# rgl-epfl/large-steps-pytorch

Measured on AMD Instinct MI355X. Metric: from_differential_solves_per_sec, higher is better.
Workload: dtype f32; 1 GPU; cfg4_plane1m: 1000x1000 plane, V=1000000, nnz(M)=6992002, M=I+50*L_uniform, u=M v, k=3, factor once (not timed), re-solve timed; method=nested-dissection, device=AMD Radeon Graphics

## Files before the change

large-steps-pytorch_amd/csrc/direct.hip:

```cpp
#include "common.h"
#include <vector>
#include <chrono>
#include <algorithm>
#include <atomic>
#include <string.h>
#include <memory>
#include <mutex>

namespace ls {

struct alignas(64) Tile {
    int store;
    int row0, s, b, own_start, bnd_off, front_off;
    int leaf;
    int pfront_off, cix;
    int forward;
    int arity;
    long long finv_off, w_off;
};

static_assert(sizeof(Tile) == 64, "Tile layout");
__device__ __forceinline__ Tile load_tile(const Tile* __restrict__ tiles, int idx) {
    const int lane = threadIdx.x & 63;
    const int w = lane < 16 ? reinterpret_cast<const int*>(tiles)[(size_t)idx * 16 + lane] : 0;
// ... 1128 lines not shown
        p.s_cap = std::max(p.s_cap, T.nd[i].s); p.b_cap = std::max(p.b_cap, T.nd[i].b);
        red_up = std::max(red_up, T.nd[i].s); red_down = std::max(red_down, T.nd[i].s + T.nd[i].b);
    }
    p.up_b = red_up >= long_up; p.down_b = red_down >= env.long_red;
    const int up_bw = std::min(ND_BW, red_up >= 1400 ? 8 : 4), down_bw = std::min(ND_BW, red_down >= 1400 ? 8 : 4);
    p.up_nw = p.up_b ? up_bw : pick_nw(red_up, 32); p.down_nw = p.down_b ? down_bw : pick_nw(red_down, env.steps);
    int64_t rows_up = 0, rows_down = 0;
    for (int64_t i = a0; i < a1; ++i) { rows_up += T.nd[i].b; rows_down += T.nd[i].s; }
    auto pick_chunks = [&](int64_t rows, int bw) {
        int c = 4;
        while (c > 1 && rows / (ND_ROWS * bw * c) < 500) --c;
        return c;
    };
    p.up_chunks = pick_chunks(rows_up, up_bw);
    p.down_chunks = pick_chunks(rows_down, down_bw);
    const int up_rows = p.up_b ? ND_ROWS * up_bw * p.up_chunks : WAVE, down_rows = p.down_b ? ND_ROWS * down_bw * p.down_chunks : WAVE;
    const size_t up_s_bytes = ((size_t)p.s_cap * p.b_cap + (size_t)p.s_cap * kmax) * sizeof(float);
    p.up_s = p.b_cap <= 256 && p.s_cap <= 256 && up_s_bytes <= 40 * 1024 && !env.no_small;
    if (p.up_s) { p.up_b = 0; p.up_nw = std::max(1, div_up(p.b_cap, WAVE)); }
    p.up_p = !env.no_pack && p.b_cap <= WAVE && p.s_cap <= 256 && lv > 0;
    p.down_p = !env.no_pack && p.s_cap <= WAVE / 2;
    auto pack_level = [&](bool up_sweep, int& first, int& count, int& lds_rows_s, int& lds_rows_b) {
        first = (int)T.ptiles.size();
        lds_rows_s = lds_rows_b = 0;
        int64_t i = a0;
        while (i < a1) {
            PackedTile t;
            memset(&t, 0, sizeof(t));
            t.leaf = lv + 1 >= T.levels; t.arity = T.arity;
            int rows = 0;
            while (i < a1 && t.n < ND_PACK) {
                const NodeD& nd = T.nd[i];
                const int r = up_sweep ? nd.b : nd.s;
                if (t.n && rows + r > WAVE) break;
                NodeP& q = t.d[t.n];
                q.s = nd.s; q.b = nd.b; q.own_start = nd.own_start; q.bnd_off = nd.bnd_off; q.front_off = nd.front_off;
                q.pfront_off = nd.pfront_off; q.cix = nd.cix; q.pad = 0; q.finv_off = nd.finv_off; q.w_off = nd.w_off;
                t.row0[t.n + 1] = t.row0[t.n] + r;
                t.sb0[t.n + 1] = t.sb0[t.n] + nd.s;
                t.sx0[t.n + 1] = t.sx0[t.n] + nd.b;
                rows += r; ++t.n; ++i;
            }
            for (int c = t.n + 1; c <= ND_PACK; ++c) { t.row0[c] = t.row0[t.n]; t.sb0[c] = t.sb0[t.n]; t.sx0[c] = t.sx0[t.n]; }
            lds_rows_s = std::max(lds_rows_s, t.sb0[t.n]); lds_rows_b = std::max(lds_rows_b, t.sx0[t.n]);
            T.ptiles.push_back(t);
        }
        count = (int)T.ptiles.size() - first;
    };
    int dummy = 0;
    if (p.up_p) { pack_level(true, p.up_p_first, p.up_p_tiles, p.up_p_lds, dummy); p.up_s = 0; p.up_b = 0; }
    if (p.down_p) { pack_level(false, p.down_p_first, p.down_p_tiles, p.down_p_s, p.down_p_lds); p.down_b = 0; }
    p.up_first = (int)tiles.size();
    const int up_threads = WAVE * p.up_nw;
    std::vector<int> up_nodes;
    for (int64_t i = a0; i < a1; ++i) {
        const bool store_tiles = !p.up_s && T.nd[i].s > 2 * up_threads;
        const int rows = std::max(T.nd[i].b, (T.nd[i].s && !store_tiles) ? 1 : 0);
        for (int r = 0; r < rows; r += (p.up_s ? 1 << 30 : up_rows)) {
            tiles.push_back(tile_of(i, r, 0));
            tiles.back().store = (r == 0 && !store_tiles) ? 1 : 0;
            up_nodes.push_back((int)(i - a0));
        }
        if (store_tiles)
            for (int r = 0; r < T.nd[i].s; r += up_threads) { tiles.push_back(tile_of(i, r, 0)); tiles.back().store = 2; up_nodes.push_back((int)(i - a0)); }
    }
    auto xcd_order = [&](int first, std::vector<int>& node_of_tile) {
        const int n = (int)tiles.size() - first;
        if (a1 - a0 < 8 || n < 16) return;
        std::vector<std::vector<Tile>> bucket(8);
        for (int t = 0; t < n; ++t) bucket[(size_t)(node_of_tile[(size_t)t] & 7)].push_back(tiles[(size_t)(first + t)]);
        size_t longest = 0;
        for (auto& bk : bucket) longest = std::max(longest, bk.size());
        Tile idle;
        memset(&idle, 0, sizeof(idle));
        idle.store = 3; idle.forward = 2;
        tiles.resize((size_t)first);
        for (size_t r = 0; r < longest; ++r)
            for (int x = 0; x < 8; ++x) tiles.push_back(r < bucket[(size_t)x].size() ? bucket[(size_t)x][r] : idle);
    };
    xcd_order(p.up_first, up_nodes);
    p.up_tiles = (int)tiles.size() - p.up_first;
    p.down_first = (int)tiles.size();
    std::vector<int> down_nodes;
    for (int64_t i = a0; i < a1; ++i)
        for (int r = 0; r < T.nd[i].s; r += down_rows) { tiles.push_back(tile_of(i, r, 0)); down_nodes.push_back((int)(i - a0)); }
    if (lv + 1 < T.levels)
        for (int64_t i = a0; i < a1; ++i)
            for (int r = 0; r < T.nd[i].b; r += WAVE * p.down_nw) { tiles.push_back(tile_of(i, r, 1)); down_nodes.push_back((int)(i - a0)); }
    xcd_order(p.down_first, down_nodes);
    p.down_tiles = (int)tiles.size() - p.down_first;
    return ((size_t)p.s_cap + p.b_cap + 16 * WAVE) * kmax * sizeof(float);
}

void account_index_bytes(const CreatePlan& T, ls_direct* d) {
    const int levels = T.levels, arity = T.arity;
    d->lvl_idx_up.assign((size_t)levels, 0); d->lvl_idx_down.assign((size_t)levels, 0);
    std::vector<int64_t> fpos((size_t)levels, 0), bsum((size_t)levels + 1, 0);
    for (int lv = 0; lv < levels; ++lv)
        for (int64_t i = T.level_off[lv]; i < T.level_off[lv + 1]; ++i)
            if (T.active(i, lv)) { fpos[(size_t)lv] += T.nd[i].s + T.nd[i].b; bsum[(size_t)lv] += T.nd[i].b; }
    for (int lv = 0; lv < d->tier_root; ++lv) {
        const LevelPlan& p = d->plan[lv];
        d->lvl_idx_up[(size_t)lv] = (p.up_p ? (int64_t)p.up_p_tiles * (int64_t)sizeof(PackedTile) : (int64_t)p.up_tiles * (int64_t)sizeof(Tile)) + fpos[(size_t)lv] + 4 * bsum[(size_t)lv];
        d->lvl_idx_down[(size_t)lv] = (p.down_p ? (int64_t)p.down_p_tiles * (int64_t)sizeof(PackedTile) : (int64_t)p.down_tiles * (int64_t)sizeof(Tile)) + 4 * fpos[(size_t)lv] +
                                      4 * bsum[(size_t)lv + 1];
    }
    if (d->tier_root >= levels) return;
    const int H = levels - d->tier_root;
    for (const TierWG& g : T.wgs)
        for (int ph = 0; ph < H; ++ph) {
            d->lvl_idx_up[(size_t)(levels - 1 - ph)] += (int64_t)(g.up_off[ph + 1] - g.up_off[ph]) * (int64_t)sizeof(TierItem);
            d->lvl_idx_down[(size_t)(d->tier_root + ph)] += (int64_t)(g.down_off[ph + 1] - g.down_off[ph]) * (int64_t)sizeof(TierItem);
        }
    d->lvl_idx_up[(size_t)d->tier_root] += (int64_t)T.wgs.size() * (int64_t)sizeof(TierWG);
    d->lvl_idx_down[(size_t)d->tier_root] += (int64_t)T.wgs.size() * (int64_t)sizeof(TierWG);
    for (int lv = d->tier_root; lv < levels; ++lv) {
        const bool inner = lv + 1 < levels;
        if (inner) d->lvl_idx_up[(size_t)lv] += 4 * (int64_t)arity * fpos[(size_t)lv];
        if (lv == d->tier_root || !inner) d->lvl_idx_up[(size_t)lv] += 4 * bsum[(size_t)lv];
        if (inner) d->lvl_idx_down[(size_t)lv] += 4 * fpos[(size_t)lv] + 4 * bsum[(size_t)lv + 1];
    }
    const int64_t q0 = T.sub_lo * T.span(T.cut, d->tier_root);
    double mx[2] = {0, 0}, sum[2] = {0, 0};
    for (size_t w = 0; w < T.wgs.size(); ++w) {
        double wu = 0, wd = 0;
        int64_t span = 1;
        for (int lv = d->tier_root; lv < levels; ++lv) {
            const int64_t first = T.level_off[lv] + (q0 + (int64_t)w) * span;
            for (int64_t i = first; i < first + span; ++i) {
                const NodeD& n = T.nd[i];
                const double s4 = (n.s + 3) & ~3, b4 = (n.b + 3) & ~3, tri_w = ((int64_t)n.s * (n.s + 1) / 2 + 3) & ~(int64_t)3;
                if (n.flags & NODE_SPARSE) { wu += tri_w + 3.0 * n.b; wd += tri_w + 3.0 * n.b; }
                else { wu += s4 * n.b; wd += (s4 + b4) * n.s; }
            }
            span *= arity;
        }
        mx[0] = std::max(mx[0], wu); mx[1] = std::max(mx[1], wd); sum[0] += wu; sum[1] += wd;
    }
    const double nw = (double)std::max<size_t>(T.wgs.size(), 1);
    d->tier_balance[0] = mx[0]; d->tier_balance[1] = sum[0] / nw; d->tier_balance[2] = mx[1]; d->tier_balance[3] = sum[1] / nw;
}

}

extern "C" int ls_direct_create(const ls_direct_arrays* A, int device, void* stream, ls_direct** out) {
    LS_REQUIRE(A && out, LS_E_INVALID, "ls_direct_create: null argument");
    LS_REQUIRE(A->tier_waves == 0 || A->tier_waves == TIER_WAVES || A->tier_waves == TIER_WAVES_WIDE || A->tier_waves == TIER_WAVES_FULL, LS_E_INVALID,
               "ls_direct_create: tier_waves must be 0 (library's rule), 4, 8 or 16");
    const int64_t V = A->V, n_bnd = A->n_bnd, n_front = A->n_front;
    const int levels = A->levels, arity = A->arity;
    LS_REQUIRE(A->h_nodes && A->h_perm && A->h_push_ptr && V > 0 && levels >= 1 && levels <= 30 && n_bnd >= 0 && n_front >= V &&
               (arity == 2 || arity == 4 || arity == 8), LS_E_INVALID, "ls_direct_create: bad argument");
    LS_REQUIRE(V < INT32_MAX && n_bnd < INT32_MAX && n_front * arity < INT32_MAX, LS_E_OVERFLOW, "ls_direct_create: plan exceeds int32 offsets");
    *out = nullptr;
    CreatePlan T{levels, arity};
    T.level_off.resize((size_t)levels + 1);
    {
        int64_t cnt = 1, off = 1;
        for (int lv = 0; lv <= levels; ++lv) {
            T.level_off[lv] = off; off += cnt; cnt *= arity;
            LS_REQUIRE(off < ((int64_t)1 << 30), LS_E_OVERFLOW, "ls_direct_create: tree too large");
        }
    }
    DeviceGuard g(device);
    LS_HIP(g.err);
    hipStream_t st = (hipStream_t)stream;
    const bool timing = env_plan_timing();
    const NdEnv env = nd_env();
    const auto t_create = std::chrono::steady_clock::now();
    auto lap = [&](const char* what) { if (timing) fprintf(stderr, "[ls_direct_create] %-28s %.2f ms\n", what, std::chrono::duration<double, std::milli>(std::chrono::steady_clock::now() - t_create).count()); };
    std::unique_ptr<ls_direct, int (*)(ls_direct*)> d(new ls_direct(), ls_direct_destroy);
    d->device = device; d->levels = levels; d->arity = arity; d->n_nodes = (int)(T.level_off[levels] - 1); d->V = V; d->n_bnd = n_bnd; d->n_front = n_front;
    d->finv = A->d_finv; d->wf = A->d_wf; d->wb = A->d_wb;
    d->u4 = A->d_u4; d->d4 = A->d_d4;
    d->tri = A->d_tri; d->sp_ptr = A->d_sp_ptr; d->sp_ent = (const SpEnt*)A->d_sp_ent;
    const int n_ranks = std::max(1, (int)A->shard_count), rank = std::min(std::max(0, (int)A->shard_rank), n_ranks - 1);
    int cut = 0;
    while (cut + 1 < levels && T.level_off[cut + 1] - T.level_off[cut] < n_ranks) ++cut;
    if (n_ranks == 1) cut = 0;
    const int64_t n_sub = T.level_off[cut + 1] - T.level_off[cut];
    T.sub_lo = n_sub * rank / n_ranks; T.sub_hi = n_sub * (rank + 1) / n_ranks;
    d->shard_rank = rank; d->shard_count = n_ranks; d->cut = T.cut = cut;
    T.mask.assign((size_t)n_front, 0);
    int rc = LS_OK;
    if ((rc = read_nodes(A, T, d.get())) || (rc = choose_tier(T, A->h_ppos, A->tier_waves, env, d.get()))) return rc;
    d->upper_lo = (d->tier_root < levels && d->tier_root > 0) ? T.nd[T.level_off[d->tier_root - 1]].own_start : (int)V;
    d->plan.resize(levels);
    size_t lds_max = 0;
    const int long_up = env.long_up > 0 ? env.long_up : levels >= 8 ? 256 : 64;
    for (int lv = 0; lv < d->tier_root; ++lv) lds_max = std::max(lds_max, plan_level(T, lv, long_up, env, d->kmax, d->plan[lv]));
    account_index_bytes(T, d.get());
    if (lds_max > LEVEL_LDS) {
        set_error("ls_direct_create: a front needs %zu bytes of LDS (separator too large for this kernel)", lds_max);
        return LS_E_INVALID;
    }
    if (n_ranks > 1 && cut >= 1) {
        d->exch_f0 = T.nd[T.level_off[cut - 1]].front_off;
        d->exch_f1 = T.nd[T.level_off[cut]].front_off;
    }
    if (n_ranks > 1) {
        d->owned_rows.assign((size_t)V, 0);
        for (int lv = 0; lv < levels; ++lv)
            for (int64_t i = T.level_off[lv]; i < T.level_off[lv + 1]; ++i)
                if (lv < cut ? rank == 0 : T.active(i, lv))
                    for (int r = 0; r < T.nd[i].s; ++r) d->owned_rows[(size_t)A->h_perm[T.nd[i].own_start + r]] = 1;
    }
    lap("tables built (host)");
    hipStream_t su = side_stream(device, 0);
    LS_REQUIRE(su, LS_E_STATE, "ls_direct_create: no side stream on this device");
    auto table = [&](void** dst, size_t bytes) -> hipError_t {
        size_t cap = bytes;
        *dst = pool_take(device, bytes, &cap);
        if (!*dst) { const hipError_t e = pool_alloc(device, dst, bytes); if (e != hipSuccess) return e; }
        d->tables.emplace_back(*dst, cap);
        return hipSuccess;
    };
    auto up = [&](auto** dst, const auto* src, size_t n) -> int {
        LS_HIP(table((void**)dst, std::max<size_t>(n, 1) * sizeof(**dst)));
        if (n) LS_HIP(hipMemcpyAsync(*dst, src, n * sizeof(**dst), hipMemcpyHostToDevice, su));
        return LS_OK;
    };
    if ((rc = up(&d->tiles, T.tiles.data(), T.tiles.size())) || (rc = up(&d->ptiles, T.ptiles.data(), T.ptiles.size())) ||
        (rc = up(&d->perm, A->h_perm, (size_t)V)) ||
        (rc = up(&d->ppos, A->h_ppos, (size_t)n_bnd)) || (rc = up(&d->push_ptr, A->h_push_ptr, (size_t)n_front + 1)) ||
        (rc = up(&d->push_tgt, A->h_push_tgt, (size_t)n_bnd)) || (rc = up(&d->mask, T.mask.data(), T.mask.size())) ||
        (rc = up(&d->d_items, T.items.data(), T.items.size())) || (rc = up(&d->pull, T.pull.data(), T.pull.size())) ||
        (rc = up(&d->d_wgs, T.wgs.data(), T.wgs.size())))
        return rc;
    hipError_t e = table((void**)&d->bp, sizeof(float) * (size_t)V * d->kmax);
    if (e == hipSuccess) e = table((void**)&d->braw, sizeof(float) * (size_t)V * d->kmax);
    if (e == hipSuccess) e = table((void**)&d->slots, sizeof(float) * (size_t)n_front * d->arity * d->kmax);
    if (e == hipSuccess) e = table((void**)&d->xb, sizeof(float) * (size_t)std::max<int64_t>(n_bnd, 1) * d->kmax);
    if (e == hipSuccess) e = hipEventCreateWithFlags(&d->busy, hipEventDisableTiming);
    lap("uploads enqueued, vectors allocated");
    if (e == hipSuccess) e = hipEventRecord(d->busy, su);
    if (e == hipSuccess) e = hipStreamWaitEvent(st, d->busy, 0);
    if (e == hipSuccess) e = hipStreamSynchronize(su);
    lap("uploads done");
    if (e != hipSuccess) return hip_fail(e, "ls_direct_create allocations", __FILE__, __LINE__);
    static const void* const kernels[] = {
#define LS_OPTIN(KK)                                                                                                                \
        (const void*)k_nd_up<KK, false>, (const void*)k_nd_down<KK, false>, (const void*)k_nd_up_b<KK, false>,                      \
        (const void*)k_nd_down_b<KK, false>, (const void*)k_nd_up<KK, true>, (const void*)k_nd_down<KK, true>,                      \
        (const void*)k_nd_up_b<KK, true>, (const void*)k_nd_down_b<KK, true>, (const void*)k_nd_up_s<KK>,
        LS_OPTIN(1) LS_OPTIN(2) LS_OPTIN(3) LS_OPTIN(4)
#undef LS_OPTIN
#define LS_OPTIN(KK)                                                                                                                \
        (const void*)k_nd_tier<KK, true, TIER_WAVES, false>, (const void*)k_nd_tier<KK, false, TIER_WAVES, false>,                  \
        (const void*)k_nd_tier<KK, true, TIER_WAVES, true>, (const void*)k_nd_tier<KK, false, TIER_WAVES, true>,                    \
        (const void*)k_nd_tier<KK, true, TIER_WAVES_WIDE, false>, (const void*)k_nd_tier<KK, false, TIER_WAVES_WIDE, false>,        \
        (const void*)k_nd_tier<KK, true, TIER_WAVES_FULL, false>, (const void*)k_nd_tier<KK, false, TIER_WAVES_FULL, false>,        \
        (const void*)k_nd_tier<KK, true, TIER_WAVES_FULL, true>, (const void*)k_nd_tier<KK, false, TIER_WAVES_FULL, true>,
        LS_OPTIN(1) LS_OPTIN(2) LS_OPTIN(3) LS_OPTIN(4)
#undef LS_OPTIN
    };
    for (const void* k : kernels) (void)hipFuncSetAttribute(k, hipFuncAttributeMaxDynamicSharedMemorySize, LDS_OPTIN);
    lap("kernel attributes set");
    *out = d.release();
    return LS_OK;
}

extern "C" int ls_direct_destroy(ls_direct* d) {
    if (!d) return LS_OK;
    DeviceGuard g(d->device);
    if (d->busy) (void)hipEventDestroy(d->busy);
    if (!d->tables.empty()) (void)hipDeviceSynchronize();
    for (const auto& t : d->tables)
        if (!ls::pool_give(d->device, t.first, t.second)) (void)hipFree(t.first);
    ls::refactor_state_free(d->refac);
    for (hipEvent_t e : d->ev) (void)hipEventDestroy(e);
#ifdef LS_TIER_STAMPS
    if (d->stamps) (void)hipFree(d->stamps);
#endif
    for (hipEvent_t e : d->lev) (void)hipEventDestroy(e);
    delete d;
    return LS_OK;
}

template <int K>
static int direct_solve_k(ls_direct* d, const float* b, float* x, hipStream_t st, int part, float* exchange) {
    const int top = d->tier_root - 1;
    TierArgs ta;
    ta.items = d->d_items; ta.wgs = d->d_wgs; ta.perm = d->perm; ta.mask = d->mask; ta.ppos = d->ppos;
    ta.pull = d->pull ? d->pull - (size_t)d->pull_base * d->arity : nullptr; ta.push_ptr = d->push_ptr; ta.push_tgt = d->push_tgt; ta.u4 = d->u4; ta.d4 = d->d4; ta.tri = d->tri;
    ta.sp_ptr = d->sp_ptr; ta.sp_ent = d->sp_ent; ta.bprime = d->bp; ta.braw = d->braw; ta.slots = d->slots; ta.xb = d->xb;
    ta.arity = d->arity; ta.phases = d->tier_phases; ta.region_floats = d->tier_region; ta.vec_floats = d->tier_vec;
    ta.upper_lo = d->upper_lo; ta.upper_hi = (int)d->V;
#ifdef LS_TIER_STAMPS
    const size_t stamp_n = (size_t)d->tier_wgs * d->tier_waves * TIER_STAMP_SLOTS;
    if (d->profile == 2 && !d->stamps && stamp_n) LS_HIP(hipMalloc((void**)&d->stamps, 2 * stamp_n * sizeof(long long)));
    if (d->profile == 2 && d->stamps) LS_HIP(hipMemsetAsync(d->stamps, 0, 2 * stamp_n * sizeof(long long), st));
    ta.stamps = d->profile == 2 ? d->stamps : nullptr;
#endif
    const size_t tier_lds = (size_t)d->tier_region * d->tier_waves * sizeof(float);
    const bool nt_tier = d->nt_tier && d->tier_waves != TIER_WAVES_WIDE, nt = d->nt_levels;
    int n_mark = 0;
    auto mark = [&](int lo, int hi, int sweep) -> hipError_t {
        if (d->profile != 3) return hipSuccess;
        while ((int)d->lev.size() <= n_mark + 1) { hipEvent_t e; const hipError_t r = hipEventCreate(&e); if (r != hipSuccess) return r; d->lev.push_back(e); }
        if ((int)d->lmeta.size() <= n_mark) d->lmeta.resize((size_t)n_mark + 1);
        d->lmeta[(size_t)n_mark] = {lo, hi, sweep};
        return hipEventRecord(d->lev[(size_t)n_mark++], st);
    };
    auto mark_end = [&]() -> hipError_t {
        if (d->profile != 3) return hipSuccess;
        hipError_t r = hipEventRecord(d->lev[(size_t)n_mark], st);
// ... 321 lines not shown
```

large-steps-pytorch_amd/csrc/nd_tier.h:

```cpp
#pragma once

namespace ls {

constexpr int TIER_MAX_H = 6;
constexpr int TIER_WAVES = 4;
constexpr int TIER_WAVES_WIDE = 8;
constexpr int TIER_WAVES_FULL = 16;
constexpr int TIER_LDS_FULL = 160 * 1024;
constexpr int TIER_LDS = 150 * 1024;
constexpr int TIER_LDS_WIDE = 80 * 1024;
constexpr int LEVEL_LDS = 150 * 1024;
constexpr int LDS_OPTIN = 160 * 1024;
constexpr int TIER_TRI4 = 9;
constexpr int TIER_SPE = 4;

enum : int { NODE_LEAF = 1, NODE_SPARSE = 2, NODE_QUAD = 4, NODE_UPC = 8 };

struct SpEnt { float val; int idx; };

struct NodeD {
    int s, b, own_start, bnd_off, front_off, pfront_off, cix, flags;
    long long finv_off, w_off;
    int spb_off, sps_off;
};

struct alignas(32) TierItem {
    int s, b, own_start, bnd_off, front_off, pfront_off, cix, flags;
    long long finv_off, w_off;
    int spb_off, sps_off;
    int row0, r0, r1, part, nparts, pad0, pad1, pad2;
};
static_assert(sizeof(TierItem) == 96, "TierItem layout");

struct alignas(64) TierWG {
    int up_off[TIER_MAX_H + 1];
    int down_off[TIER_MAX_H + 1];
    unsigned up_split, down_split;
    unsigned up_leaf, down_leaf;
    int n_dense, pad;
    int dense_rng[2 * TIER_MAX_H];
};
static_assert(sizeof(TierWG) == 128, "TierWG layout (read as 32 dwords)");

struct TierArgs {
    const TierItem* items;
    const TierWG* wgs;
    const int* perm;
    const unsigned char* mask;
    const int* ppos;
    const int* pull;
    const int* push_ptr;
    const int* push_tgt;
    const float* u4;
    const float* d4;
    const float* tri;
    const int* sp_ptr;
    const SpEnt* sp_ent;
    float* bprime;
    int upper_lo, upper_hi;
    float* braw;
    float* slots;
    float* xb;
    int arity, phases, region_floats, vec_floats;
#ifdef LS_TIER_STAMPS
    long long* stamps;
#endif
};

constexpr int TIER_STAMP_SLOTS = 32;
#ifdef LS_TIER_STAMPS
#define LS_STAMP(slot) do { if (a.stamps && lane == 0) stamp_base[(slot)] = (long long)wall_clock64(); } while (0)
#define LS_STAMP_VAL(slot, v) do { if (a.stamps && lane == 0) stamp_base[(slot)] = (long long)(v); } while (0)
#else
#define LS_STAMP(slot) do { } while (0)
#define LS_STAMP_VAL(slot, v) do { } while (0)
#endif

constexpr int ITEM_DWORDS = 24;
__device__ __forceinline__ int rec_load(const TierItem* items, int k, int lane) {
    return lane < ITEM_DWORDS ? reinterpret_cast<const int*>(items)[(size_t)k * ITEM_DWORDS + lane] : 0;
}
__device__ __forceinline__ int rl(int v, int i) { return __builtin_amdgcn_readlane(v, i); }
__device__ __forceinline__ TierItem rec_unpack(int r) {
    TierItem t;
    t.s = rl(r, 0); t.b = rl(r, 1); t.own_start = rl(r, 2); t.bnd_off = rl(r, 3); t.front_off = rl(r, 4); t.pfront_off = rl(r, 5);
    t.cix = rl(r, 6); t.flags = rl(r, 7);
    t.finv_off = (long long)(((unsigned long long)(unsigned)rl(r, 9) << 32) | (unsigned)rl(r, 8));
    t.w_off = (long long)(((unsigned long long)(unsigned)rl(r, 11) << 32) | (unsigned)rl(r, 10));
    t.spb_off = rl(r, 12); t.sps_off = rl(r, 13); t.row0 = rl(r, 14); t.r0 = rl(r, 15); t.r1 = rl(r, 16); t.part = rl(r, 17);
    t.nparts = rl(r, 18); t.pad0 = t.pad1 = t.pad2 = 0;
    return t;
}

__device__ __forceinline__ void wave_lds_sync() {
    __builtin_amdgcn_fence(__ATOMIC_RELEASE, "wavefront");
    __builtin_amdgcn_wave_barrier();
    __builtin_amdgcn_fence(__ATOMIC_ACQUIRE, "wavefront");
}

__device__ __forceinline__ float bcast_lane(float v, int c) {
    return __int_as_float(__builtin_amdgcn_readlane(__float_as_int(v), c));
}

template <int K>
__device__ __forceinline__ void pull_compact(const TierArgs& a, size_t f, float (&v)[K]) {
#pragma unroll
    for (int q = 0; q < K; ++q) v[q] = 0.0f;
    const int* pl = a.pull + f * a.arity;
    for (int c = 0; c < a.arity; ++c) {
        const int idx = pl[c];
        if (idx >= 0) {
#pragma unroll
            for (int q = 0; q < K; ++q) v[q] += a.xb[(size_t)idx * K + q];
        }
    }
}

template <int K>
__device__ __forceinline__ void pull_values(const TierArgs& a, const int (&pl)[4], float (&v)[K]) {
#pragma unroll
    for (int q = 0; q < K; ++q) v[q] = 0.0f;
#pragma unroll
    for (int c = 0; c < 4; ++c) {
        if (pl[c] >= 0) {
#pragma unroll
            for (int q = 0; q < K; ++q) v[q] += a.xb[(size_t)pl[c] * K + q];
        }
    }
}
__device__ __forceinline__ void pull_indices(const TierArgs& a, size_t f, bool on, int (&pl)[4]) {
#pragma unroll
    for (int c = 0; c < 4; ++c) pl[c] = on ? a.pull[f * 4 + c] : -1;
}

struct LeafIdx {
    int g, p0, p1, pp;
};
template <int K>
struct LeafDat {
    float4 t[TIER_TRI4];
    float v[K];
    float xv[K];
    SpEnt e[TIER_SPE];
};

template <bool UP>
__device__ __forceinline__ void leaf_idx(const TierArgs& a, const TierItem& n, int lane, LeafIdx& ix) {
    ix.g = lane < n.s ? a.perm[n.own_start + lane] : 0;
    if (UP) {
        const bool r = lane < n.b;
        ix.p0 = r ? a.sp_ptr[n.spb_off + lane] : 0;
        ix.p1 = r ? a.sp_ptr[n.spb_off + lane + 1] : 0;
        ix.pp = r ? a.ppos[n.bnd_off + lane] : 0;
    } else {
        const bool r = lane < n.s;
        ix.p0 = r ? a.sp_ptr[n.sps_off + lane] : 0;
        ix.p1 = r ? a.sp_ptr[n.sps_off + lane + 1] : 0;
        ix.pp = 0;
    }
}

template <int K, bool UP, bool NT>
__device__ __forceinline__ void leaf_dat(const TierArgs& a, const TierItem& n, const LeafIdx& ix, const float* __restrict__ b_in,
                                         int lane, LeafDat<K>& d) {
    if (!UP) {
#pragma unroll
        for (int q = 0; q < K; ++q) d.xv[q] = lane < n.b ? a.xb[(size_t)(n.bnd_off + lane) * K + q] : 0.0f;
    }
    const float2* __restrict__ ent = reinterpret_cast<const float2*>(a.sp_ent);
    if (!UP) {
#pragma unroll
        for (int t = 0; t < TIER_SPE; ++t) {
            const bool ok = ix.p0 + t < ix.p1;
            const float2 r = ld_stream2<NT>(ent + (ok ? ix.p0 + t : 0));
            d.e[t].val = ok ? r.x : 0.0f;
            d.e[t].idx = ok ? __float_as_int(r.y) : 0;
        }
    }
    const float4* __restrict__ p = reinterpret_cast<const float4*>(a.tri + n.finv_off);
    const int n4 = (n.s * (n.s + 1) / 2 + 3) >> 2;
#pragma unroll
    for (int e = 0; e < TIER_TRI4; ++e) {
        const int i = lane + e * 64;
        d.t[e] = i < n4 ? p[i] : make_float4(0.f, 0.f, 0.f, 0.f);
    }
#pragma unroll
    for (int q = 0; q < K; ++q) {
        if (UP) d.v[q] = lane < n.s ? b_in[(size_t)ix.g * K + q] : 0.0f;
        else d.v[q] = lane < n.s ? a.bprime[(size_t)(n.own_start + lane) * K + q] : 0.0f;
    }
    if (UP) {
#pragma unroll
        for (int t = 0; t < TIER_SPE; ++t) {
            const bool ok = ix.p0 + t < ix.p1;
            const float2 r = ld_stream2<NT>(ent + (ok ? ix.p0 + t : 0));
            d.e[t].val = ok ? r.x : 0.0f;
            d.e[t].idx = ok ? __float_as_int(r.y) : 0;
        }
    }
}

template <int K>
__device__ __forceinline__ void tri_stage(const LeafDat<K>& d, int s, int lane, float* stage) {
    float4* o = reinterpret_cast<float4*>(stage);
    const int n4 = (s * (s + 1) / 2 + 3) >> 2;
#pragma unroll
    for (int e = 0; e < TIER_TRI4; ++e) {
        const int i = lane + e * 64;
        if (i < n4) o[i] = d.t[e];
    }
}

typedef float f32x4 __attribute__((ext_vector_type(4)));

template <int E>
__device__ __forceinline__ f32x4 mv_step(float vec16, float m, f32x4 acc) {
    return __builtin_amdgcn_mfma_f32_4x4x1f32(vec16, m, acc, 4, E, 0);
}

template <int C>
__device__ __forceinline__ float tri_select(float lo, float hi) {
    if (C == 0) return lo;
    unsigned long long mask;
    asm volatile("s_lshl_b64 %0, -1, %1" : "=s"(mask) : "n"(C) : "scc");
    return __builtin_amdgcn_inverse_ballot_w64(mask) ? lo : hi;
}
template <int T, int E>
__device__ __forceinline__ float tri_element(const float* stage, int j, int tj) {
    constexpr int c = 16 * T + E;
    const float lo = stage[tj + c];
    if (c == 0) return lo;
    const float hi = stage[c * (c + 1) / 2 + j];
    return tri_select<c>(lo, hi);
}
template <int T>
__device__ __forceinline__ void tri_chunk(const float* stage, const float* vec4, int s, int lane, int j, int tj, f32x4& a0, f32x4& a1) {
    if (16 * T >= s) return;
    const float v16 = vec4[64 * T + lane];
    float m[16];
    {
    m[0] = tri_element<T, 0>(stage, j, tj);   m[1] = tri_element<T, 1>(stage, j, tj);   m[2] = tri_element<T, 2>(stage, j, tj);   m[3] = tri_element<T, 3>(stage, j, tj);
    m[4] = tri_element<T, 4>(stage, j, tj);   m[5] = tri_element<T, 5>(stage, j, tj);   m[6] = tri_element<T, 6>(stage, j, tj);   m[7] = tri_element<T, 7>(stage, j, tj);
    m[8] = tri_element<T, 8>(stage, j, tj);   m[9] = tri_element<T, 9>(stage, j, tj);   m[10] = tri_element<T, 10>(stage, j, tj); m[11] = tri_element<T, 11>(stage, j, tj);
    m[12] = tri_element<T, 12>(stage, j, tj); m[13] = tri_element<T, 13>(stage, j, tj); m[14] = tri_element<T, 14>(stage, j, tj); m[15] = tri_element<T, 15>(stage, j, tj);
    }
    a0 = mv_step<0>(v16, m[0], a0);   a1 = mv_step<1>(v16, m[1], a1);   a0 = mv_step<2>(v16, m[2], a0);   a1 = mv_step<3>(v16, m[3], a1);
    a0 = mv_step<4>(v16, m[4], a0);   a1 = mv_step<5>(v16, m[5], a1);   a0 = mv_step<6>(v16, m[6], a0);   a1 = mv_step<7>(v16, m[7], a1);
    a0 = mv_step<8>(v16, m[8], a0);   a1 = mv_step<9>(v16, m[9], a1);   a0 = mv_step<10>(v16, m[10], a0); a1 = mv_step<11>(v16, m[11], a1);
    a0 = mv_step<12>(v16, m[12], a0); a1 = mv_step<13>(v16, m[13], a1); a0 = mv_step<14>(v16, m[14], a0); a1 = mv_step<15>(v16, m[15], a1);
}
template <int K>
__device__ __forceinline__ void tri_matvec(const float* stage, const float* vec4, int s, int lane, float (&acc)[K]) {
    const int j = min(lane, s - 1);
    const int tj = j * (j + 1) / 2;
    f32x4 a0 = {0.f, 0.f, 0.f, 0.f}, a1 = {0.f, 0.f, 0.f, 0.f};
    tri_chunk<0>(stage, vec4, s, lane, j, tj, a0, a1);
    tri_chunk<1>(stage, vec4, s, lane, j, tj, a0, a1);
    tri_chunk<2>(stage, vec4, s, lane, j, tj, a0, a1);
    tri_chunk<3>(stage, vec4, s, lane, j, tj, a0, a1);
#pragma unroll
    for (int q = 0; q < K; ++q) acc[q] = a0[q] + a1[q];
}

template <int K>
__device__ __forceinline__ void sparse_row(const TierArgs& a, const LeafIdx& ix, const SpEnt (&e)[TIER_SPE], const float* vec4, float (&u)[K]) {
#pragma unroll
    for (int q = 0; q < K; ++q) u[q] = 0.0f;
#pragma unroll
    for (int t = 0; t < TIER_SPE; ++t) {
        if (ix.p0 + t < ix.p1) {
#pragma unroll
            for (int q = 0; q < K; ++q) u[q] = fmaf(e[t].val, vec4[e[t].idx * 4 + q], u[q]);
        }
    }
    for (int p = ix.p0 + TIER_SPE; p < ix.p1; ++p) {
        const SpEnt z = a.sp_ent[p];
#pragma unroll
        for (int q = 0; q < K; ++q) u[q] = fmaf(z.val, vec4[z.idx * 4 + q], u[q]);
    }
}

template <int K>
// ... 60 lines not shown
    wave_lds_sync();
    sparse_row<K>(a, ix, e, xbv, t);
    wave_lds_sync();
}

template <int K>
__device__ __forceinline__ void leaf_down_vec(const TierItem& n, const float (&t)[K], float* region, int tri_floats) {
    const int lane = threadIdx.x & 63;
    float4 w = make_float4(0.f, 0.f, 0.f, 0.f);
    if (lane < n.s) { w.x = t[0]; if (K > 1) w.y = t[K > 1 ? 1 : 0]; if (K > 2) w.z = t[K > 2 ? 2 : 0]; if (K > 3) w.w = t[K > 3 ? 3 : 0]; }
    reinterpret_cast<float4*>(region + tri_floats)[lane] = w;
}

template <int K>
__device__ __forceinline__ void leaf_down_tail(const TierItem& n, const LeafIdx& ix, const float (&yj)[K], float* __restrict__ x_out,
                                               float* region, int tri_floats) {
    const int lane = threadIdx.x & 63, s = n.s;
    float z[K];
    tri_matvec<K>(region, region + tri_floats, s, lane, z);
    if (lane < s) {
#pragma unroll
        for (int q = 0; q < K; ++q) x_out[(size_t)ix.g * K + q] = yj[q] - z[q];
    }
    wave_lds_sync();
}

template <int K, bool UP, int W, bool NT>
__device__ __forceinline__ void leaf_phase(const TierArgs& a, int k0, int k1, const float* __restrict__ b_in, float* __restrict__ x_out,
                                           float* region, int tri_floats, long long* stamp_base) {
    const int lane = threadIdx.x & 63;
    int leaf_no = 0;
    (void)leaf_no; (void)stamp_base;
    if (k0 >= k1) return;
    constexpr int S = W;
    TierItem it = rec_unpack(rec_load(a.items, k0, lane));
    int rec_n = k0 + S < k1 ? rec_load(a.items, k0 + S, lane) : 0;
    LeafIdx ix;
    leaf_idx<UP>(a, it, lane, ix);
    for (int k = k0; k < k1; k += S) {
        float v[K];
        SpEnt e[TIER_SPE];
        float t[K];
        {
            LeafDat<K> d;
            leaf_dat<K, UP, NT>(a, it, ix, b_in, lane, d);
            if (!UP) leaf_down_head<K>(a, it, ix, d.xv, d.e, region, t);
            tri_stage<K>(d, it.s, lane, region);
#pragma unroll
            for (int q = 0; q < K; ++q) v[q] = d.v[q];
#pragma unroll
            for (int u = 0; u < TIER_SPE; ++u) e[u] = d.e[u];
        }
        if (!UP) leaf_down_vec<K>(it, t, region, tri_floats);
        wave_lds_sync();
        const bool more = k + S < k1;
        TierItem it_n = it;
        LeafIdx ix_n = ix;
        if (more) { it_n = rec_unpack(rec_n); leaf_idx<UP>(a, it_n, lane, ix_n); }
        rec_n = k + 2 * S < k1 ? rec_load(a.items, k + 2 * S, lane) : 0;
        if (UP) leaf_up_compute<K>(a, it, ix, v, e, region, tri_floats);
        else leaf_down_tail<K>(it, ix, v, x_out, region, tri_floats);
        if (leaf_no < 8) LS_STAMP(16 + leaf_no);
        ++leaf_no;
        it = it_n; ix = ix_n;
    }
}

#ifndef LS_TIER_Q
#define LS_TIER_Q 4
#endif
constexpr int TIER_Q = LS_TIER_Q;

template <bool NT>
__device__ __forceinline__ void tier_prefetch(const float4* __restrict__ col, size_t rows, int q0, int q1, float4 (&cur)[TIER_Q]) {
#pragma unroll
    for (int e = 0; e < TIER_Q; ++e) cur[e] = (q0 + e < q1) ? ld_stream4<NT>(col + (size_t)(q0 + e) * rows) : make_float4(0.f, 0.f, 0.f, 0.f);
}

__device__ __forceinline__ void tier_mv16(float v16, const float4& a, const float4& b, const float4& c, const float4& d, int n, f32x4& acc) {
    acc = mv_step<0>(v16, a.x, acc); acc = mv_step<1>(v16, a.y, acc); acc = mv_step<2>(v16, a.z, acc); acc = mv_step<3>(v16, a.w, acc);
    if (n > 1) { acc = mv_step<4>(v16, b.x, acc); acc = mv_step<5>(v16, b.y, acc); acc = mv_step<6>(v16, b.z, acc); acc = mv_step<7>(v16, b.w, acc); }
    if (n > 2) { acc = mv_step<8>(v16, c.x, acc); acc = mv_step<9>(v16, c.y, acc); acc = mv_step<10>(v16, c.z, acc); acc = mv_step<11>(v16, c.w, acc); }
    if (n > 3) { acc = mv_step<12>(v16, d.x, acc); acc = mv_step<13>(v16, d.y, acc); acc = mv_step<14>(v16, d.z, acc); acc = mv_step<15>(v16, d.w, acc); }
}

__device__ __forceinline__ void tier_mv_batch(const float* sv4, int base, int q, int q1, const float4 (&c)[TIER_Q], f32x4& acc) {
    const int lane = threadIdx.x & 63;
    const float4 z = make_float4(0.f, 0.f, 0.f, 0.f);
    if (TIER_Q == 2) tier_mv16(sv4[(4 * q - base) * 4 + lane], c[0], c[1], z, z, min(2, q1 - q), acc);
    if (TIER_Q >= 4) tier_mv16(sv4[(4 * q - base) * 4 + lane], c[0], c[1], c[TIER_Q >= 4 ? 2 : 0], c[TIER_Q >= 4 ? 3 : 0], q1 - q, acc);
    if (TIER_Q >= 8 && q + 4 < q1) tier_mv16(sv4[(4 * q + 16 - base) * 4 + lane], c[TIER_Q >= 8 ? 4 : 0], c[TIER_Q >= 8 ? 5 : 0],
                                             c[TIER_Q >= 8 ? 6 : 0], c[TIER_Q >= 8 ? 7 : 0], q1 - q - 4, acc);
}
template <bool NT>
__device__ __forceinline__ void tier_dot(const float4* __restrict__ col, size_t rows, int q0, int q1, const float* sv4, int base,
                                         float4 (&A)[TIER_Q], float4 (&B)[TIER_Q], f32x4& acc) {
    for (int q = q0; q < q1; q += 2 * TIER_Q) {
        tier_mv_batch(sv4, base, q, q1, A, acc);
        tier_prefetch<NT>(col, rows, q + 2 * TIER_Q, q1, A);
        if (q + TIER_Q < q1) tier_mv_batch(sv4, base, q + TIER_Q, q1, B, acc);
        tier_prefetch<NT>(col, rows, q + 3 * TIER_Q, q1, B);
    }
}

template <int K>
__device__ __forceinline__ void node_up_finish(const TierArgs& a, const TierItem& n, int i, int pp, const float (&acc)[K]) {
    if (i >= n.b || n.pfront_off < 0) return;
    if (n.flags & NODE_UPC) {
#pragma unroll
        for (int q = 0; q < K; ++q) a.xb[(size_t)(n.bnd_off + i) * K + q] = acc[q];
        return;
    }
    const size_t dst = ((size_t)(n.pfront_off + pp) * a.arity + n.cix) * K;
#pragma unroll
    for (int q = 0; q < K; ++q) a.slots[dst + q] = acc[q];
}

template <int K>
struct DensePre {
    float4 cur[TIER_Q];
    float v[K];
    int idx;
    int plo[4], plb[4];
    int fw0, fw1;
};

__device__ __forceinline__ void fwd_slice(const TierItem& it, int& f0, int& f1) {
    const int chunks = (max(it.s, 1) + 63) >> 6, total = chunks * it.nparts, ord = (it.row0 >> 6) * it.nparts + it.part;
    f0 = (int)((long long)it.b * ord / total);
    f1 = (int)((long long)it.b * (ord + 1) / total);
}

template <int K, bool NT>
__device__ __forceinline__ void node_up_pre(const TierArgs& a, const TierItem& it, DensePre<K>& P) {
    const int lane = threadIdx.x & 63, i = it.row0 + lane;
    const bool row = i < it.b;
    const float4* col = reinterpret_cast<const float4*>(a.u4 + it.w_off) + (row ? i : 0);
    tier_prefetch<NT>(col, (size_t)it.b, it.r0 >> 2, row ? it.r1 >> 2 : it.r0 >> 2, P.cur);
    const bool fin = it.part == 0 && row && it.pfront_off >= 0;
    P.idx = (fin && !(it.flags & NODE_UPC)) ? a.ppos[it.bnd_off + i] : 0;
    const bool inner = !(it.flags & NODE_LEAF) && a.arity == 4;
    const int j = it.r0 + lane;
    pull_indices(a, (size_t)(it.front_off + j), inner && j < it.r1 && j < it.s, P.plo);
    if (K <= 3) pull_indices(a, (size_t)(it.front_off + it.s + i), inner && fin, P.plb);
}

template <int K, bool NT>
__device__ __forceinline__ void node_up(const TierArgs& a, const TierItem& it, DensePre<K>& P, const float* __restrict__ b_in, float* region, float* pbuf) {
    const int lane = threadIdx.x & 63, b = it.b;
    const int i = it.row0 + lane;
    const bool row = i < b;
    float* sv4 = region;
    const float4* __restrict__ col = reinterpret_cast<const float4*>(a.u4 + it.w_off) + (row ? i : 0);
    float4 B[TIER_Q];
    tier_prefetch<NT>(col, (size_t)b, (it.r0 >> 2) + TIER_Q, it.r1 >> 2, B);
    float pass[K];
#pragma unroll
    for (int q = 0; q < K; ++q) pass[q] = 0.0f;
    const bool fin = it.part == 0 && row && it.pfront_off >= 0;
    const bool pre4 = a.arity == 4;
    if (fin && !(it.flags & NODE_LEAF)) {
        if (pre4 && K <= 3) pull_values<K>(a, P.plb, pass); else pull_compact<K>(a, (size_t)(it.front_off + it.s + i), pass);
    }
    for (int j = it.r0 + lane; j < it.r1; j += 64) {
        float v[K];
        if (j >= it.s) {
#pragma unroll
            for (int q = 0; q < K; ++q) sv4[(j - it.r0) * 4 + q] = 0.0f;
            continue;
        }
        if (it.flags & NODE_LEAF) {
            const size_t g = (size_t)a.perm[it.own_start + j];
#pragma unroll
            for (int q = 0; q < K; ++q) v[q] = b_in[g * K + q];
        } else {
#pragma unroll
            for (int q = 0; q < K; ++q) v[q] = a.braw[(size_t)(it.own_start + j) * K + q];
        }
        if (!(it.flags & NODE_LEAF)) {
            float u[K];
            if (pre4 && j == it.r0 + lane) pull_values<K>(a, P.plo, u); else pull_compact<K>(a, (size_t)(it.front_off + j), u);
#pragma unroll
            for (int q = 0; q < K; ++q) v[q] -= u[q];
        }
#pragma unroll
        for (int q = 0; q < K; ++q) sv4[(j - it.r0) * 4 + q] = v[q];
        if (it.row0 == 0) {
#pragma unroll
            for (int q = 0; q < K; ++q) a.bprime[(size_t)(it.own_start + j) * K + q] = v[q];
        }
    }
    wave_lds_sync();
    f32x4 a4 = {0.f, 0.f, 0.f, 0.f};
    tier_dot<NT>(col, (size_t)b, it.r0 >> 2, it.r1 >> 2, sv4, it.r0, P.cur, B, a4);
    float acc[K];
#pragma unroll
    for (int q = 0; q < K; ++q) acc[q] = a4[q];
    if (it.nparts == 1) {
        if (fin) {
            const bool upc = it.flags & NODE_UPC;
            const size_t dst = upc ? (size_t)(it.bnd_off + i) * K : ((size_t)(it.pfront_off + P.idx) * a.arity + it.cix) * K;
            float* out = upc ? a.xb : a.slots;
#pragma unroll
            for (int q = 0; q < K; ++q) out[dst + q] = acc[q] + pass[q];
        }
    } else {
#pragma unroll
        for (int q = 0; q < K; ++q) pbuf[lane * 4 + q] = acc[q] + pass[q];
    }
    wave_lds_sync();
}

template <int K>
__device__ __forceinline__ void node_down_store(const TierArgs& a, const TierItem& it, int g, int p0, int p1, const int (&tg)[4],
                                                float* __restrict__ x_out, const float (&acc)[K]) {
    const int j = it.row0 + (threadIdx.x & 63);
    if (j >= it.s) return;
#pragma unroll
    for (int q = 0; q < K; ++q) x_out[(size_t)g * K + q] = acc[q];
    if (it.flags & NODE_LEAF) return;
#pragma unroll
    for (int c = 0; c < 4; ++c) {
        if (tg[c] >= 0) {
#pragma unroll
            for (int q = 0; q < K; ++q) a.xb[(size_t)tg[c] * K + q] = acc[q];
        }
    }
    if (p1 - p0 > 4) push_down<K>(a.push_tgt, p0 + 4, p1, a.xb, acc);
}

template <int K>
__device__ __forceinline__ void node_down_finish(const TierArgs& a, const TierItem& it, float* __restrict__ x_out, const float (&acc)[K]) {
    const int j = it.row0 + (threadIdx.x & 63);
    if (j >= it.s) return;
    const size_t g = (size_t)a.perm[it.own_start + j];
#pragma unroll
    for (int q = 0; q < K; ++q) x_out[g * K + q] = acc[q];
    if (!(it.flags & NODE_LEAF)) push_down<K>(a.push_tgt, a.push_ptr[it.front_off + j], a.push_ptr[it.front_off + j + 1], a.xb, acc);
}

template <int K, bool NT>
__device__ __forceinline__ void node_down_pre(const TierArgs& a, const TierItem& it, DensePre<K>& P) {
    const int lane = threadIdx.x & 63, s = it.s, j = it.row0 + lane;
    const bool row = j < s;
    tier_prefetch<NT>(reinterpret_cast<const float4*>(a.d4 + it.finv_off) + (row ? j : 0), (size_t)s, it.r0 >> 2, row ? it.r1 >> 2 : it.r0 >> 2, P.cur);
    const int t = it.r0 + lane;
#pragma unroll
    for (int q = 0; q < K; ++q) P.v[q] = (t < it.r1 && t < s) ? a.bprime[(size_t)(it.own_start + t) * K + q] : 0.0f;
    const bool fin = it.part == 0 && row;
    const bool push = fin && !(it.flags & NODE_LEAF);
    P.idx = fin ? a.perm[it.own_start + j] : 0;
    P.plo[0] = push ? a.push_ptr[it.front_off + j] : 0;
    P.plo[1] = push ? a.push_ptr[it.front_off + j + 1] : 0;
    int f0, f1;
    fwd_slice(it, f0, f1);
    const bool fw = !(it.flags & NODE_LEAF) && f0 + lane < f1;
    P.fw0 = fw ? a.push_ptr[it.front_off + s + f0 + lane] : 1;
    P.fw1 = fw ? a.push_ptr[it.front_off + s + f0 + lane + 1] : 0;
}

template <int K, bool NT>
__device__ __forceinline__ void node_down(const TierArgs& a, const TierItem& it, DensePre<K>& P, float* __restrict__ x_out, float* region, float* pbuf) {
    const int lane = threadIdx.x & 63, s = it.s;
    const int j = it.row0 + lane;
    const bool row = j < s;
    float* sv4 = region;
    const float4* __restrict__ col = reinterpret_cast<const float4*>(a.d4 + it.finv_off) + (row ? j : 0);
    float4 B[TIER_Q];
    tier_prefetch<NT>(col, (size_t)s, (it.r0 >> 2) + TIER_Q, it.r1 >> 2, B);
    int f0, f1;
    fwd_slice(it, f0, f1);
    const bool fw = P.fw0 <= P.fw1;
    float fv[K];
    int ftg[2];
#pragma unroll
    for (int q = 0; q < K; ++q) fv[q] = fw ? a.xb[(size_t)(it.bnd_off + f0 + lane) * K + q] : 0.0f;
#pragma unroll
    for (int c = 0; c < 2; ++c) ftg[c] = (fw && P.fw0 + c < P.fw1) ? a.push_tgt[P.fw0 + c] : -1;
    const int s4 = (s + 3) & ~3;
    for (int t = it.r0 + lane; t < it.r1; t += 64) {
        float v[K];
        if (t < s) {
            if (t == it.r0 + lane) {
#pragma unroll
                for (int q = 0; q < K; ++q) v[q] = P.v[q];
            } else {
#pragma unroll
                for (int q = 0; q < K; ++q) v[q] = a.bprime[(size_t)(it.own_start + t) * K + q];
            }
        } else if (t >= s4 && t - s4 < it.b) {
#pragma unroll
            for (int q = 0; q < K; ++q) v[q] = -a.xb[(size_t)(it.bnd_off + t - s4) * K + q];
        } else {
#pragma unroll
            for (int q = 0; q < K; ++q) v[q] = 0.0f;
        }
#pragma unroll
        for (int q = 0; q < K; ++q) sv4[(t - it.r0) * 4 + q] = v[q];
    }
    wave_lds_sync();
#pragma unroll
    for (int c = 0; c < 4; ++c) P.plb[c] = (it.nparts == 1 && P.plo[0] + c < P.plo[1]) ? a.push_tgt[P.plo[0] + c] : -1;
    f32x4 a4 = {0.f, 0.f, 0.f, 0.f};
    tier_dot<NT>(col, (size_t)s, it.r0 >> 2, it.r1 >> 2, sv4, it.r0, P.cur, B, a4);
    float acc[K];
#pragma unroll
    for (int q = 0; q < K; ++q) acc[q] = a4[q];
    if (it.nparts == 1) node_down_store<K>(a, it, P.idx, P.plo[0], P.plo[1], P.plb, x_out, acc);
    else {
#pragma unroll
        for (int q = 0; q < K; ++q) pbuf[lane * 4 + q] = acc[q];
    }
#pragma unroll
    for (int c = 0; c < 2; ++c) {
        if (ftg[c] >= 0) {
#pragma unroll
            for (int q = 0; q < K; ++q) a.xb[(size_t)ftg[c] * K + q] = fv[q];
        }
    }
    if (fw && P.fw1 - P.fw0 > 2) push_down<K>(a.push_tgt, P.fw0 + 2, P.fw1, a.xb, fv);
    if (!(it.flags & NODE_LEAF)) {
        for (int i = f0 + 64 + lane; i < f1; i += 64) {
            const size_t f = (size_t)(it.front_off + s + i);
            const int p0 = a.push_ptr[f], p1 = a.push_ptr[f + 1];
            float v[K];
#pragma unroll
            for (int q = 0; q < K; ++q) v[q] = a.xb[(size_t)(it.bnd_off + i) * K + q];
            push_down<K>(a.push_tgt, p0, p1, a.xb, v);
        }
    }
    wave_lds_sync();
}

template <int K, bool UP, int W, bool NT>
__global__ __launch_bounds__(64 * W, 16 / W) void k_nd_tier(TierArgs a, const float* __restrict__ b_in, float* __restrict__ x_out,
                                                              int tri_floats) {
    extern __shared__ __attribute__((aligned(16))) float sm[];
    const int wave = __builtin_amdgcn_readfirstlane(threadIdx.x >> 6), lane = threadIdx.x & 63;
    float* region = sm + (size_t)wave * a.region_floats;
    for (int i = lane; 4 * i < a.region_floats; i += 64) reinterpret_cast<float4*>(region)[i] = make_float4(0.f, 0.f, 0.f, 0.f);
    wave_lds_sync();
    const int n_wg = (int)gridDim.x;
    const int sub = __builtin_expect((n_wg & 7) == 0, 1) ? (int)(blockIdx.x & 7) * (n_wg >> 3) + (int)(blockIdx.x >> 3) : (int)blockIdx.x;
#ifdef LS_TIER_STAMPS
    long long* stamp_base = a.stamps ? a.stamps + ((size_t)sub * W + wave) * TIER_STAMP_SLOTS : nullptr;
#else
    long long* stamp_base = nullptr;
#endif
    LS_STAMP(0);
    const int hdr = lane < 32 ? reinterpret_cast<const int*>(a.wgs + sub)[lane] : 0;
    const int obase = UP ? 0 : TIER_MAX_H + 1;
    const unsigned split = (unsigned)rl(hdr, UP ? 14 : 15), leafy = (unsigned)rl(hdr, UP ? 16 : 17);
    if (UP) {
        const int n_dense = rl(hdr, 18);
        for (int r = threadIdx.x; r < n_dense; r += blockDim.x) {
            int o = r, start = 0;
#pragma unroll
            for (int t = 0; t < TIER_MAX_H; ++t) {
                const int cnt = rl(hdr, 20 + 2 * t + 1);
                const bool here = o >= 0 && o < cnt;
                start = here ? rl(hdr, 20 + 2 * t) + o : start;
                o = here ? -1 : o - cnt;
            }
            const size_t g = (size_t)a.perm[start];
#pragma unroll
            for (int q = 0; q < K; ++q) a.braw[(size_t)start * K + q] = b_in[g * K + q];
        }
        for (int r = a.upper_lo + blockIdx.x * blockDim.x + threadIdx.x; r < a.upper_hi; r += gridDim.x * blockDim.x) {
            const size_t g = (size_t)a.perm[r];
#pragma unroll
            for (int q = 0; q < K; ++q) a.braw[(size_t)r * K + q] = b_in[g * K + q];
        }
    }
    LS_STAMP(1);
    DensePre<K> pre;
#pragma unroll
    for (int e = 0; e < TIER_Q; ++e) pre.cur[e] = make_float4(0.f, 0.f, 0.f, 0.f);
#pragma unroll
    for (int q = 0; q < K; ++q) pre.v[q] = 0.0f;
    pre.idx = 0; pre.fw0 = 1; pre.fw1 = 0;
#pragma unroll
    for (int c = 0; c < 4; ++c) { pre.plo[c] = -1; pre.plb[c] = -1; }
    TierItem it_pre = rec_unpack(0);
    bool pre_valid = false;
    for (int ph = 0; ph < a.phases; ++ph) {
        const int i0 = rl(hdr, obase + ph), i1 = rl(hdr, obase + ph + 1);
        int rec_nx = 0;
        bool has_nx = false;
        if (ph + 1 < a.phases && !((leafy >> (ph + 1)) & 1u)) {
            const int j0 = rl(hdr, obase + ph + 1) + wave;
            has_nx = j0 < rl(hdr, obase + ph + 2);
            if (has_nx) rec_nx = rec_load(a.items, j0, lane);
        }
        if ((leafy >> ph) & 1u) {
            leaf_phase<K, UP, W, NT>(a, i0 + wave, i1, b_in, x_out, region, tri_floats, stamp_base);
        } else {
            int rec = (!pre_valid && i0 + wave < i1) ? rec_load(a.items, i0 + wave, lane) : 0;
            int head_k = -1, head_idx = 0, head_p0 = 0, head_p1 = 0, head_flags = 0;
            for (int k = i0 + wave; k < i1; k += W) {
                const int rec_next = k + W < i1 ? rec_load(a.items, k + W, lane) : 0;
                const bool first = k == i0 + wave && pre_valid;
                const TierItem it = first ? it_pre : rec_unpack(rec);
                rec = rec_next;
                float* pbuf = region + a.vec_floats + ((k - i0) / W) * 256;
                if (!first) { if (UP) node_up_pre<K, NT>(a, it, pre); else node_down_pre<K, NT>(a, it, pre); }
                if (UP) node_up<K, NT>(a, it, pre, b_in, region, pbuf);
                else node_down<K, NT>(a, it, pre, x_out, region, pbuf);
                if (it.nparts > 1 && it.part == 0) {
                    head_k = k; head_idx = pre.idx; head_p0 = pre.plo[0]; head_p1 = pre.plo[1]; head_flags = it.flags;
                }
            }
            if ((split >> ph) & 1u) {
                const int rec_head = head_k >= 0 ? rec_load(a.items, head_k, lane) : 0;
                int head_tg[4];
#pragma unroll
                for (int c = 0; c < 4; ++c) head_tg[c] = (!UP && head_k >= 0 && head_p0 + c < head_p1 && !(head_flags & NODE_LEAF)) ? a.push_tgt[head_p0 + c] : -1;
                __syncthreads();
                for (int k = i0 + wave; k < i1; k += W) {
                    const bool mine = k == head_k;
                    const TierItem it = rec_unpack(mine ? rec_head : rec_load(a.items, k, lane));
                    if (it.nparts == 1 || it.part != 0) continue;
                    float acc[K];
#pragma unroll
                    for (int q = 0; q < K; ++q) acc[q] = 0.0f;
                    for (int p = 0; p < it.nparts; ++p) {
                        const int kp = k + p - i0;
                        const float* pb = sm + (size_t)(kp % W) * a.region_floats + a.vec_floats + (kp / W) * 256;
#pragma unroll
                        for (int q = 0; q < K; ++q) acc[q] += pb[lane * 4 + q];
                    }
                    if (UP) {
                        const int i = it.row0 + lane;
                        const int pp = mine ? head_idx : ((i < it.b && it.pfront_off >= 0 && !(it.flags & NODE_UPC)) ? a.ppos[it.bnd_off + i] : 0);
                        node_up_finish<K>(a, it, i, pp, acc);
                    } else if (mine) {
                        node_down_store<K>(a, it, head_idx, head_p0, head_p1, head_tg, x_out, acc);
                    }
                    else node_down_finish<K>(a, it, x_out, acc);
                }
            }
        }
        if (ph < 6) { LS_STAMP(2 + 2 * ph); LS_STAMP_VAL(24 + ph, (i1 - i0 - wave + W - 1) / W); }
        pre_valid = has_nx;
        it_pre = rec_unpack(rec_nx);
        if (pre_valid) {
            if (UP) node_up_pre<K, NT>(a, it_pre, pre); else node_down_pre<K, NT>(a, it_pre, pre);
        } else {
#pragma unroll
            for (int e = 0; e < TIER_Q; ++e) pre.cur[e] = make_float4(0.f, 0.f, 0.f, 0.f);
#pragma unroll
            for (int q = 0; q < K; ++q) pre.v[q] = 0.0f;
            pre.idx = 0; pre.fw0 = 1; pre.fw1 = 0;
#pragma unroll
            for (int c = 0; c < 4; ++c) { pre.plo[c] = -1; pre.plb[c] = -1; }
        }
        __syncthreads();
        if (ph < 6) LS_STAMP(3 + 2 * ph);
    }
}

}
```

Before: 5220 solves/s.

## Batch unconditional child gathers and hoist inner-node pulls in tier up-sweep

Replaces the branchy per-child gather loop with unconditional clamped-index loads issued together, then a predicated sum, so several independent global loads can be in flight at once instead of being serialized behind branches. In node_up, the first own-row braw load and the pull gathers for boundary and own rows are issued early, before the loop. Adds a 32-bit offset check at create time so 32-bit address arithmetic is safe. It also changes launch_bounds min-blocks for narrower waves, which alters the register budget. The cost is extra loads of xb[0] for missing children and higher register pressure.

Result: faster. 5277 solves/s, median of 6 (+1.1%).

```diff
diff --git a/large-steps-pytorch_amd/csrc/direct.hip b/large-steps-pytorch_amd/csrc/direct.hip
--- a/large-steps-pytorch_amd/csrc/direct.hip
+++ b/large-steps-pytorch_amd/csrc/direct.hip
@@ -1304,6 +1304,7 @@
     LS_REQUIRE(A->h_nodes && A->h_perm && A->h_push_ptr && V > 0 && levels >= 1 && levels <= 30 && n_bnd >= 0 && n_front >= V &&
                (arity == 2 || arity == 4 || arity == 8), LS_E_INVALID, "ls_direct_create: bad argument");
     LS_REQUIRE(V < INT32_MAX && n_bnd < INT32_MAX && n_front * arity < INT32_MAX, LS_E_OVERFLOW, "ls_direct_create: plan exceeds int32 offsets");
+    LS_REQUIRE(n_bnd * (int64_t)(4 * sizeof(float)) <= (int64_t)UINT32_MAX, LS_E_OVERFLOW, "ls_direct_create: boundary vectors exceed 4 GB");
     *out = nullptr;
     CreatePlan T{levels, arity};
     T.level_off.resize((size_t)levels + 1);
diff --git a/large-steps-pytorch_amd/csrc/nd_tier.h b/large-steps-pytorch_amd/csrc/nd_tier.h
--- a/large-steps-pytorch_amd/csrc/nd_tier.h
+++ b/large-steps-pytorch_amd/csrc/nd_tier.h
@@ -102,32 +102,50 @@
     return __int_as_float(__builtin_amdgcn_readlane(__float_as_int(v), c));
 }
 
+template <int K, int N>
+__device__ __forceinline__ void pull_request(const TierArgs& a, const int (&pl)[N], float (&r)[N][K]) {
+    const char* base = reinterpret_cast<const char*>(a.xb);
+#pragma unroll
+    for (int c = 0; c < N; ++c) {
+        const float* p = reinterpret_cast<const float*>(base + (unsigned)max(pl[c], 0) * (unsigned)(K * sizeof(float)));
+#pragma unroll
+        for (int q = 0; q < K; ++q) r[c][q] = p[q];
+    }
+}
+template <int K, int N>
+__device__ __forceinline__ void pull_sum(const int (&pl)[N], const float (&r)[N][K], float (&v)[K]) {
+#pragma unroll
+    for (int c = 0; c < N; ++c) {
+#pragma unroll
+        for (int q = 0; q < K; ++q) v[q] = pl[c] >= 0 ? v[q] + r[c][q] : v[q];
+    }
+}
+
+template <int K, int A>
+__device__ __forceinline__ void pull_compact_n(const TierArgs& a, size_t f, float (&v)[K]) {
+    constexpr int G = A * K <= 16 ? A : 4;
+    int pl[A];
+#pragma unroll
+    for (int c = 0; c < A; ++c) pl[c] = a.pull[f * A + c];
+#pragma unroll
+    for (int c0 = 0; c0 < A; c0 += G) {
+        int pg[G];
+        float r[G][K];
+#pragma unroll
+        for (int c = 0; c < G; ++c) pg[c] = pl[c0 + c];
+        pull_request<K, G>(a, pg, r);
+        pull_sum<K, G>(pg, r, v);
+    }
+}
 template <int K>
 __device__ __forceinline__ void pull_compact(const TierArgs& a, size_t f, float (&v)[K]) {
 #pragma unroll
     for (int q = 0; q < K; ++q) v[q] = 0.0f;
-    const int* pl = a.pull + f * a.arity;
-    for (int c = 0; c < a.arity; ++c) {
-        const int idx = pl[c];
-        if (idx >= 0) {
-#pragma unroll
-            for (int q = 0; q < K; ++q) v[q] += a.xb[(size_t)idx * K + q];
-        }
-    }
-}
-
-template <int K>
-__device__ __forceinline__ void pull_values(const TierArgs& a, const int (&pl)[4], float (&v)[K]) {
-#pragma unroll
-    for (int q = 0; q < K; ++q) v[q] = 0.0f;
-#pragma unroll
-    for (int c = 0; c < 4; ++c) {
-        if (pl[c] >= 0) {
-#pragma unroll
-            for (int q = 0; q < K; ++q) v[q] += a.xb[(size_t)pl[c] * K + q];
-        }
-    }
-}
+    if (a.arity == 4) pull_compact_n<K, 4>(a, f, v);
+    else if (a.arity == 8) pull_compact_n<K, 8>(a, f, v);
+    else pull_compact_n<K, 2>(a, f, v);
+}
+
 __device__ __forceinline__ void pull_indices(const TierArgs& a, size_t f, bool on, int (&pl)[4]) {
 #pragma unroll
     for (int c = 0; c < 4; ++c) pl[c] = on ? a.pull[f * 4 + c] : -1;
@@ -494,15 +512,27 @@
     const bool row = i < b;
     float* sv4 = region;
     const float4* __restrict__ col = reinterpret_cast<const float4*>(a.u4 + it.w_off) + (row ? i : 0);
+    const bool fin = it.part == 0 && row && it.pfront_off >= 0;
+    const bool inner = !(it.flags & NODE_LEAF);
+    const bool pre4 = a.arity == 4 && inner;
     float4 B[TIER_Q];
     tier_prefetch<NT>(col, (size_t)b, (it.r0 >> 2) + TIER_Q, it.r1 >> 2, B);
-    float pass[K];
-#pragma unroll
-    for (int q = 0; q < K; ++q) pass[q] = 0.0f;
-    const bool fin = it.part == 0 && row && it.pfront_off >= 0;
-    const bool pre4 = a.arity == 4;
-    if (fin && !(it.flags & NODE_LEAF)) {
-        if (pre4 && K <= 3) pull_values<K>(a, P.plb, pass); else pull_compact<K>(a, (size_t)(it.front_off + it.s + i), pass);
+    const int j0 = it.r0 + lane;
+    const bool own0 = pre4 && j0 < it.r1 && j0 < it.s;
+    float pass[K], u0[K], v0[K];
+#pragma unroll
+    for (int q = 0; q < K; ++q) pass[q] = u0[q] = v0[q] = 0.0f;
+    if (pre4) {
+        float rb[4][K], ro[4][K];
+        if (K <= 3) pull_request<K, 4>(a, P.plb, rb);
+        else if (fin) pull_compact_n<K, 4>(a, (size_t)(it.front_off + it.s + i), pass);
+        pull_request<K, 4>(a, P.plo, ro);
+#pragma unroll
+        for (int q = 0; q < K; ++q) v0[q] = a.braw[(size_t)(own0 ? it.own_start + j0 : 0) * K + q];
+        if (K <= 3) pull_sum<K, 4>(P.plb, rb, pass);
+        pull_sum<K, 4>(P.plo, ro, u0);
+    } else if (fin && inner) {
+        pull_compact<K>(a, (size_t)(it.front_off + it.s + i), pass);
     }
     for (int j = it.r0 + lane; j < it.r1; j += 64) {
         float v[K];
@@ -515,13 +545,15 @@
             const size_t g = (size_t)a.perm[it.own_start + j];
 #pragma unroll
             for (int q = 0; q < K; ++q) v[q] = b_in[g * K + q];
+        } else if (pre4 && j == j0) {
+#pragma unroll
+            for (int q = 0; q < K; ++q) v[q] = v0[q] - u0[q];
         } else {
+            const size_t f = (size_t)(it.front_off + j);
 #pragma unroll
             for (int q = 0; q < K; ++q) v[q] = a.braw[(size_t)(it.own_start + j) * K + q];
-        }
-        if (!(it.flags & NODE_LEAF)) {
             float u[K];
-            if (pre4 && j == it.r0 + lane) pull_values<K>(a, P.plo, u); else pull_compact<K>(a, (size_t)(it.front_off + j), u);
+            pull_compact<K>(a, f, u);
 #pragma unroll
             for (int q = 0; q < K; ++q) v[q] -= u[q];
         }
@@ -675,7 +707,7 @@
 }
 
 template <int K, bool UP, int W, bool NT>
-__global__ __launch_bounds__(64 * W, 16 / W) void k_nd_tier(TierArgs a, const float* __restrict__ b_in, float* __restrict__ x_out,
+__global__ __launch_bounds__(64 * W, W >= 16 ? 1 : 4) void k_nd_tier(TierArgs a, const float* __restrict__ b_in, float* __restrict__ x_out,
                                                               int tri_floats) {
     extern __shared__ __attribute__((aligned(16))) float sm[];
     const int wave = __builtin_amdgcn_readfirstlane(threadIdx.x >> 6), lane = threadIdx.x & 63;
```
